# melspectrum007/audio-visual-speech-enhancement

Measured on AMD Instinct MI355X. Metric: clips/sec (STFT+CNN forward) on 200-ms@16kHz segments, 1/2/4/8 MI355X, higher is better.
Workload: dtype fp32_split

## Files before the change

audio-visual-speech-enhancement_amd/csrc/avse_common.h:

```cpp
#pragma once
#include <hip/hip_runtime.h>
#include <stdint.h>
#include <string>

#include "layer_geom.h"
#include "options.h"

typedef __bf16 bf16_t;
typedef __bf16 bf16x8 __attribute__((ext_vector_type(8)));
typedef _Float16 f16x8 __attribute__((ext_vector_type(8)));
typedef _Float16 f16x4 __attribute__((ext_vector_type(4)));
typedef float f32x4 __attribute__((ext_vector_type(4)));
typedef int i32x4 __attribute__((ext_vector_type(4)));

struct avse_ctx;

namespace avse {

void set_error(const std::string& msg);

int ctx_device_index(const struct ::avse_ctx* c);

int ensure_lds_attr(const void* fn, int bytes);

// ... 166 lines not shown
    const float* sh4;
    int nt4, kpad4;
    int pt4, pl4, rows4, pitch4;
    int dy4, dx4, nx4;
    const bf16_t* w5;
    const float* sc5;
    const float* sh5;
    int nt5[4], kpad5[4];
    int dy5[4], dx5[4], nx5[4];
    long long woff5[4];
    int pt5, pl5, rows5, pitch5;
    const float* w6;
    float b6;
    unsigned* range_flag;
    unsigned range_bit;
};
bool dec_tail_supported(const DecTailArgs& a);
bool dec_tail_s16_supported(const DecTailArgs& a);
int launch_dec_tail_s16(const DecTailArgs& a, hipStream_t s);

struct AudEncArgs {
    const float* mel;
    bf16_t* out;
    long long out_clip_stride;
    int N;
    const bf16_t* w1;
    const bf16_t* w2;
    const bf16_t* w3;
    const bf16_t* w4;
    const bf16_t* w5;
// ... 23 lines not shown
    const bf16_t* w;
    int M, N, kpad;
    const float* scale;
    const float* shift;
    int act;
    bf16_t* out;
    long long ldo;
    int out_off;
    int ksplit;
    float* partial;
    int* counters;
    int split;
    int slabs_per_split;
    unsigned* range_flag;
    unsigned range_bit;
};
int gemm_ksplit(int M, int N, int kpad, int cap);
int gemm_s16_ksplit(int N, int kpad, int* slabs_per_split);
size_t gemm_ws_bytes(int M, int N, int kpad, int cap);
int launch_gemm(const GemmArgs& g, int mode, hipStream_t s);
int launch_aud_enc(const AudEncArgs& a, hipStream_t s);
int launch_dec_tail(const DecTailArgs& a, hipStream_t s);

enum HaloOut { OUT_BF16 = 0, OUT_S16 = 1, OUT_F32 = 2 };

struct HaloArgs {
    int variant;
    const void* in;
    const float* video;
    const float* vmean;
// ... 48 lines not shown
```

audio-visual-speech-enhancement_amd/csrc/capi.hip:

```cpp
#include <algorithm>
#include <atomic>
#include <cmath>
#include <cstdio>
#include <cstdlib>
#include <cstring>
#include <mutex>
#include <set>
#include <string>
#include <utility>
#include <vector>

#include "../../include/avse.h"
#include "avse_common.h"
#include "netplan.h"
#include "spec_tables.h"
#include "weight_pack.h"

namespace avse {
static thread_local std::string g_err;
void set_error(const std::string& msg) { g_err = msg; }

int ensure_lds_attr(const void* fn, int bytes) {
    static std::mutex mu;
    static std::set<std::pair<const void*, int>> done;
// ... 104 lines not shown
    {"no_audenc", "AVSE_NO_AUDENC", &Options::no_audenc},
    {"no_dechead", "AVSE_NO_DECHEAD", &Options::no_dechead},
    {"no_dectail", "AVSE_NO_DECTAIL", &Options::no_dectail},
    {"unfused_tail", "AVSE_UNFUSED_TAIL", &Options::unfused_tail},
    {"no_halo", "AVSE_NO_HALO", &Options::no_halo},
    {"mfma32", "AVSE_MFMA32", &Options::mfma32},
    {"serial", "AVSE_SERIAL", &Options::serial},
    {"graph", "AVSE_GRAPH", &Options::graph},
    {"gemm_ksplit_cap", "AVSE_GEMM_KSPLIT", &Options::gemm_ksplit_cap},
    {"dense_istft", "AVSE_DENSE_ISTFT", &Options::dense_istft},
    {"no_act_scale", "AVSE_NO_ACT_SCALE", &Options::no_act_scale},
    {"no_win", "AVSE_NO_WIN", &Options::no_win},
    {"no_v1p", "AVSE_NO_V1P", &Options::no_v1p},
    {"no_a1valu", "AVSE_NO_A1VALU", &Options::no_a1valu},
    {"no_planar", "AVSE_NO_PLANAR", &Options::no_planar},
    {"side_prio", "AVSE_SIDE_PRIO", &Options::side_prio},
};

struct avse_weights {
    int dtype = 0;
    int device = 0;
    uint64_t serial = 0;
    NetPlan plan = kPlan25;
    GpuLayer layers[kNumLayers - 1];
    float* d6_w = nullptr;
    float d6_bias = 0.f;
    mutable std::atomic<void*> vzero_emb{nullptr};
    mutable std::mutex vzero_mu;
    mutable unsigned vzero_range = 0;
    int act_exp[kNumLayers] = {};
// ... 340 lines not shown
const char* avse_last_error(void) { return g_err.c_str(); }

int avse_ctx_create(int device, avse_ctx** out) {
    if (!out) return fail(AVSE_ERR_INVALID, "out is NULL");
    int n = 0;
    AVSE_HIP_CHECK(hipGetDeviceCount(&n));
    if (device < 0 || device >= n) return fail(AVSE_ERR_INVALID, "bad device index");
    AVSE_HIP_CHECK(hipSetDevice(device));
    avse_ctx* c = new avse_ctx();
    c->device = device;
    for (const OptionName& o : kOptionNames) {
        const char* e = std::getenv(o.env);
        if (e && *e) c->opt.*(o.field) = std::atoi(e);
    }
    if (hipMalloc((void**)&c->mse_partial, sizeof(float) * 256) != hipSuccess ||
        hipMalloc((void**)&c->gemm_counters, sizeof(int) * 8192) != hipSuccess ||
        hipMemset(c->gemm_counters, 0, sizeof(int) * 8192) != hipSuccess ||
        hipMalloc((void**)&c->range, sizeof(unsigned) * 4) != hipSuccess ||
        hipMemset(c->range, 0, sizeof(unsigned) * 4) != hipSuccess ||
        hipHostMalloc((void**)&c->range_host, sizeof(unsigned) * 4, hipHostMallocDefault) != hipSuccess) {
        (void)hipFree(c->mse_partial);
        (void)hipFree(c->gemm_counters);
        (void)hipFree(c->range);
        delete c;
        return fail(AVSE_ERR_OOM, "hipMalloc failed (ctx)");
    }
    *out = c;
    return 0;
}

void avse_ctx_destroy(avse_ctx* c) {
    if (!c) return;
// ... 335 lines not shown
        if (split) {
            g.split = 1;
            if (mode == 1) {
                g.ksplit = choose_ksplit(g.M, g.N, g.kpad, dt);
                g.slabs_per_split = g.ksplit > 1 ? kFp32Block : 0;
            } else {
                g.ksplit = gemm_s16_ksplit(g.N, g.kpad, &g.slabs_per_split);
            }
            g.range_flag = rflag;
            g.range_bit = 1u << li;
        } else {
            g.ksplit = gemm_ksplit(g.M, g.N, g.kpad, opt.gemm_ksplit_cap);
        }
        g.partial = reinterpret_cast<float*>(c->arena + part_off);
        g.counters = c->gemm_counters;
        return launch_gemm(g, mode, s);
    };
    auto ksplit = [&](ConvArgs& a, size_t partial_off) {
        if (a.nphase != 1) return;
        const int64_t M = (int64_t)a.N * a.Hq * a.Wq;
        a.ksplit = choose_ksplit(M, a.Co, a.ph[0].kpad, dt, a.ph[0].ntaps == 1, &a.ksplit_slabs);
        a.partial = reinterpret_cast<float*>(c->arena + partial_off);
    };
    auto L = [&](int i) -> const GpuLayer& { return W->layers[i]; };
    int stage = 0;
    auto mark = [&]() -> int {
        if (ev) AVSE_HIP_CHECK(hipEventRecord(ev[stage], s));
        ++stage;
        return 0;
    };
// ... 141 lines not shown
                             : conv_args(G, buf(a_in[i]), in_cs, buf(B_CAT), CAT, G.def.cout, 0, N);
        const int dti = pairs(a, i > 0, true, i);
        if ((rc = conv(a, dti, G, sa)) || (rc = mark())) return rc;
    }
    if (concurrent) AVSE_HIP_CHECK(hipEventRecord(c->join, sa));
    if (video) {
        if ((rc = video_encoder(video, vdt, vmean, vstd, N, off, buf(B_CAT)))) return rc;
    } else {
        const size_t es = dt == AVSE_BF16 ? 2 : 4;
        if ((rc = launch_broadcast_row(W->vzero_emb.load(std::memory_order_acquire), (char*)buf(B_CAT) + AEMB * es, N, 2048 * es, CAT * es, s))) return rc;
        if (split && W->vzero_range && rflag && (rc = launch_flag_or(rflag, W->vzero_range, s))) return rc;
        for (int k = 0; k < 6; ++k)
            if ((rc = mark())) return rc;
    }
    if (concurrent) AVSE_HIP_CHECK(hipStreamWaitEvent(s, c->join, 0));
    if (use_gemm) {
        if ((rc = gemm(L(11), buf(B_CAT), CAT, buf(B_E1), EMB, 0, 0, N, off[B_COUNT], 11)) || (rc = mark())) return rc;
        if ((rc = gemm(L(12), buf(B_E1), EMB, buf(B_E2), EMB, 0, 0, N, off[B_COUNT], 12)) || (rc = mark())) return rc;
        if ((rc = gemm(L(13), buf(B_E2), EMB, buf(B_E3), AEMB, 0, 0, N, off[B_COUNT], 13)) || (rc = mark())) return rc;
    } else {
        ConvArgs a = conv_args(L(11), buf(B_CAT), CAT, buf(B_E1), EMB, EMB, 0, N);
        ksplit(a, off[B_COUNT]);
        int dti = pairs(a, true, true, 11);
        if ((rc = launch_conv(a, split ? dti : cdt, s)) || (rc = mark())) return rc;
        a = conv_args(L(12), buf(B_E1), EMB, buf(B_E2), EMB, EMB, 0, N);
        ksplit(a, off[B_COUNT]);
        dti = pairs(a, true, true, 12);
        if ((rc = launch_conv(a, split ? dti : cdt, s)) || (rc = mark())) return rc;
        a = conv_args(L(13), buf(B_E2), EMB, buf(B_E3), AEMB, AEMB, 0, N);
        ksplit(a, off[B_COUNT]);
        dti = pairs(a, true, true, 13);
        if ((rc = launch_conv(a, split ? dti : cdt, s)) || (rc = mark())) return rc;
    }
    const int d_in[6] = {B_E3, B_D1, B_D2, B_D3, B_D4, B_D5};
    for (int i = 0; i < 5; ++i) {
        const GpuLayer& G = L(14 + i);
        const long long in_cs = (long long)G.def.hin * G.def.win * G.def.cin;
        if (i == 0 && dt == AVSE_BF16) {
            auto taps_ok = [&](const GpuLayer& D, int np, int nt, bool wide) {
                if (D.nphase != np || D.def.cin != 128 || D.def.cout != 128) return false;
                for (int p = 0; p < np; ++p) {
                    if (D.ph[p].ntaps != nt || D.ph[p].kpad != nt * 128 || D.ph[p].w_off != (long long)p * 128 * nt * 128) return false;
                    for (int t = 0; t < nt; ++t) {
                        const int2 d = D.htaps[D.ph[p].tap_off + t];
                        const int dy = wide ? (p >> 1) - (t >> 1) : 0, dx = wide ? (p & 1) - (t & 1) : -t;
                        if (d.x != dy || d.y != dx) return false;
                    }
// ... 10 lines not shown
            ha.out = reinterpret_cast<bf16_t*>(buf(B_D3));
            ha.out_clip_stride = 40 * 10 * 128;
            ha.N = (int)N;
            ha.w1 = (const bf16_t*)L(14).w; ha.w2 = (const bf16_t*)L(15).w; ha.w3 = (const bf16_t*)L(16).w;
            for (int k = 0; k < 3; ++k) { ha.sc[k] = L(14 + k).scale; ha.sh[k] = L(14 + k).shift; }
            if (shapes && !opt.no_dechead && dec_head_supported(ha)) {
                if ((rc = launch_dec_head(ha, s)) || (rc = mark()) || (rc = mark()) || (rc = mark())) return rc;
                i = 2;
                continue;
            }
        }
        if (i == 3 && split && !opt.unfused_tail && !opt.no_dectail) {
            DecTailArgs da = dec_tail_args(L(17), L(18), W, buf(d_in[3]), out, N);
            da.range_flag = rflag;
            da.range_bit = 1u << 17;
            if (dec_tail_s16_supported(da)) {
                if ((rc = launch_dec_tail_s16(da, s)) || (rc = mark()) || (rc = mark())) return rc;
                break;
            }
        }
        if (i == 3 && dt == AVSE_BF16 && !opt.unfused_tail && !opt.no_dectail) {
            const DecTailArgs da = dec_tail_args(L(17), L(18), W, buf(d_in[3]), out, N);
            if (dec_tail_supported(da)) {
                if ((rc = launch_dec_tail(da, s)) || (rc = mark()) || (rc = mark())) return rc;
                break;
            }
        }
        if (i == 4 && !opt.unfused_tail) {
            ConvArgs a = conv_args(G, buf(d_in[i]), in_cs, nullptr, (long long)G.ho * G.wo, 1, 0, N);
            a.fuse_w = W->d6_w;
// ... 247 lines not shown
```

audio-visual-speech-enhancement_amd/csrc/conv_dects.hip:

```cpp
#include <cstdlib>
#include <utility>

#include "avse_common.h"

namespace avse {
namespace {

#ifndef AVSE_DECTS_ABL
#define AVSE_DECTS_ABL 0
#endif
constexpr int DABL = AVSE_DECTS_ABL;
constexpr float LRELU = 0.3f;
constexpr int kOOB = 0x7fffff00;
constexpr int H = 40, W = 10;
constexpr int CI4 = 128, CO = 64;
constexpr int NW = 8, NT = 64 * NW;
constexpr int R4 = 21;
constexpr int F4 = 14, F5 = 13, SL = 7;
constexpr int P4 = 18, S4 = 96, ROWS4 = 26, WBUF = ROWS4 * P4 * S4;
constexpr int LROWS4 = 24, LCOLS4 = 14, NPC = 3;
constexpr int P5 = 18, S5 = 288, ROWS5 = 23, OIMG = ROWS5 * P5 * S5;
constexpr int REGION = ((OIMG > 2 * WBUF ? OIMG : 2 * WBUF) + 1023) / 1024 * 1024;
constexpr int BOFF = REGION;
constexpr int PAR = BOFF + 2 * 4 * 4096;
constexpr int PSC4 = PAR, PSH4 = PAR + 256, PSC5 = PAR + 512, PSH5 = PAR + 768, PW6 = PAR + 1024;
constexpr int XP = PAR + 1280;
constexpr int LDS_BYTES = XP + 4 * 16 * F5 * 4;
static_assert(LDS_BYTES <= 160 * 1024, "LDS");
static_assert(2 * SL == F4 && 16 * F4 >= R4 * W && 16 * F5 >= H / 2 * W && 16 * (F5 - 1) < H / 2 * W, "fragments");

constexpr int ph_ny(int p) { return 2 + (p >> 1); }
constexpr int ph_nx(int p) { return 2 + (p & 1); }
constexpr int ph_nt(int p) { return ph_ny(p) * ph_nx(p); }
constexpr int ph_woff(int p) { int s = 0; for (int q = 0; q < p; ++q) s += CO * ph_nt(q) * CO; return s; }
constexpr int ph_gstart(int p) { int s = 0; for (int q = 0; q < p; ++q) s += 4 * ph_nt(q); return s; }
constexpr int ph_of(int g) { int p = 0; while (p < 3 && g >= ph_gstart(p + 1)) ++p; return p; }
static_assert(ph_gstart(4) % 4 == 0 && (4 * ph_nt(0)) % 4 == 0, "every phase is whole ring groups");

__device__ __forceinline__ __amdgpu_buffer_rsrc_t make_rsrc(const void* base, long long bytes) {
    const int nrec = bytes > kOOB ? kOOB : (bytes < 0 ? 0 : (int)bytes);
    return __builtin_amdgcn_make_buffer_rsrc(const_cast<void*>(base), (short)0, nrec, 0x00020000);
}
__device__ __forceinline__ int wsw(int row) { return 2 * ((row >> 2) & 1); }
__device__ __forceinline__ i32x4 lds16(const char* base, int off) { return *reinterpret_cast<const i32x4*>(base + off); }
typedef int i32x2 __attribute__((ext_vector_type(2)));
__device__ __forceinline__ float bn_lrelu(float acc, float sc, float sh) {
    const float v = fmaf(acc, sc, sh);
    return fmaxf(v, LRELU * v);
}
__device__ __forceinline__ void lds_barrier_raw() {
    asm volatile("s_waitcnt lgkmcnt(0)" ::: "memory");
    asm volatile("s_barrier" ::: "memory");
}
__device__ __forceinline__ void lds_barrier() { lds_barrier_raw(); }
__device__ __forceinline__ void loop_barrier() {
    if constexpr (!(DABL & 4)) lds_barrier_raw();
}
template <int... I, typename F>
__device__ __forceinline__ void unroll(std::integer_sequence<int, I...>, F&& f) {
    (f(std::integral_constant<int, I>{}), ...);
}

__global__ __launch_bounds__(NT, 1) void k_dec_tail_s16(DecTailArgs a) {
    extern __shared__ __attribute__((aligned(1024))) char lds[];

    const int tid = threadIdx.x, lane = tid & 63;
    const int w = __builtin_amdgcn_readfirstlane(tid >> 6);
    const int r16 = lane & 15, kg = lane >> 4;
    const int clip = blockIdx.x >> 1, half = blockIdx.x & 1;
    const int cb = w & 3, fr0 = SL * (w >> 2);
    const bool s6 = w < 4;

    const int brow = tid >> 3, kq = (tid >> 1) & 3, kh = tid & 1;
    const int bst = BOFF + brow * 64 + ((kq ^ wsw(brow)) << 4) + kh * 8;
    const int brd = 16 * cb + r16;
    const int bfh = BOFF + brd * 64 + (((kg & 1) ^ wsw(brd)) << 4);
    const int bfl = BOFF + brd * 64 + (((2 + (kg & 1)) ^ wsw(brd)) << 4);
    auto st8 = [&](int addr, i32x2 v) { *reinterpret_cast<i32x2*>(lds + addr) = v; };
    auto read_w = [&](int off, i32x4 (&f)[2]) {
        f[0] = lds16(lds, bfh + off);
        f[1] = lds16(lds, bfl + off);
    };

    f32x4 acc[SL], part[SL];
    auto zero_all = [&]() {
#pragma unroll
        for (int i = 0; i < SL; ++i) acc[i] = part[i] = (f32x4){0.f, 0.f, 0.f, 0.f};
    };
    auto flush = [&]() {
#pragma unroll
        for (int i = 0; i < SL; ++i) {
            acc[i] += part[i];
            part[i] = (f32x4){0.f, 0.f, 0.f, 0.f};
        }
    };
    auto mfma_all = [&](const i32x4 (&fa)[SL], const i32x4 (&fw)[2], bool slot6) {
        if constexpr (DABL & 1) {
#pragma unroll
            for (int i = 0; i < SL; ++i) asm volatile("" ::"v"(fa[i]));
            asm volatile("" ::"v"(fw[0]), "v"(fw[1]));
            return;
        }
#pragma unroll
        for (int i = 0; i < SL; ++i) {
            if (i == SL - 1 && !slot6) continue;
            part[i] = __builtin_amdgcn_mfma_f32_16x16x32_f16(__builtin_bit_cast(f16x8, fw[0]), __builtin_bit_cast(f16x8, fa[i]),
                                                             part[i], 0, 0, 0);
            part[i] = __builtin_amdgcn_mfma_f32_16x16x32_f16(__builtin_bit_cast(f16x8, fw[1]), __builtin_bit_cast(f16x8, fa[i]),
                                                             part[i], 0, 0, 0);
        }
    };
// ... 22 lines not shown
            pok[k] = p < LROWS4 * LCOLS4;
            const bool in = pok[k] && iy >= 0 && iy < H && ix >= 0 && ix < W;
            psrc[k] = in ? ((iy * W + ix) * CI4 * 2 + sg * 8) * 2 : kOOB;
            pdst[k] = (wr * P4 + wc) * S4 + sg * 16;
        }
        const __amdgpu_buffer_rsrc_t rsW = make_rsrc(a.w4, (long long)CO * 16 * CI4 * 4);
        const int vbl = brow * (16 * CI4 * 4) + kq * 16 + kh * 8;
        auto bpiece = [&](auto tt, int csoff) {
            constexpr int t = decltype(tt)::value;
            return __builtin_amdgcn_raw_buffer_load_b64(rsW, vbl + t * 512, csoff, 0);
        };
        int vb[SL];
#pragma unroll
        for (int i = 0; i < SL; ++i) {
            const int q = 16 * (fr0 + i) + r16, r = q / W, x = q - r * W;
            vb[i] = (r * P4 + x) * S4 + kg * 16;
        }
        {
            i32x4 pc[NPC];
#pragma unroll
            for (int k = 0; k < NPC; ++k) pc[k] = __builtin_amdgcn_raw_buffer_load_b128(rsIn, psrc[k], 0, 0);
#pragma unroll
            for (int k = 0; k < NPC; ++k)
                if (pok[k]) *reinterpret_cast<i32x4*>(lds + pdst[k]) = pc[k];
        }
        i32x2 pb[4];
        {
            i32x2 w0[4];
            unroll(std::make_integer_sequence<int, 4>{}, [&](auto tt) {
                constexpr int t = decltype(tt)::value;
                w0[t] = bpiece(tt, 0);
                pb[t] = bpiece(std::integral_constant<int, t + 4>{}, 0);
            });
#pragma unroll
            for (int t = 0; t < 4; ++t) st8(bst + t * 4096, w0[t]);
        }
        zero_all();
        lds_barrier();

        i32x4 fa[2][SL], fw[2][2];
        constexpr int PST = 12;
        i32x4 pr[NPC];
        int wb = 0;
        auto read_a = [&](auto tt, i32x4 (&f)[SL]) {
            constexpr int t = decltype(tt)::value % 16;
            constexpr int imm = ((3 - t / 4) * P4 + (3 - t % 4)) * S4;
#pragma unroll
            for (int i = 0; i < SL; ++i) f[i] = lds16(lds + imm + wb, vb[i]);
        };
        read_a(std::integral_constant<int, 0>{}, fa[0]);
        read_w(0, fw[0]);
        for (int c = 0; c < 8; ++c) {
            const int nb = (c & 1) ? 0 : WBUF;
            const int cs = c * 64, cn = (c + 1) * 64;
            unroll(std::make_integer_sequence<int, 16>{}, [&](auto tt) {
                constexpr int t = decltype(tt)::value;
                __builtin_amdgcn_sched_barrier(0);
                st8(bst + (((t / 4) + 1) & 1) * 16384 + (t % 4) * 4096, pb[t & 3]);
                if constexpr (t + 8 < 16) pb[t & 3] = bpiece(std::integral_constant<int, t + 8>{}, cs);
                else pb[t & 3] = bpiece(std::integral_constant<int, t + 8 - 16>{}, cn);
                if constexpr (t < NPC) pr[t] = __builtin_amdgcn_raw_buffer_load_b128(rsIn, psrc[t], cn, 0);
                if constexpr (t >= PST && t - PST < NPC) {
                    if (pok[t - PST] && c < 7) *reinterpret_cast<i32x4*>(lds + nb + pdst[t - PST]) = pr[t - PST];
                }
                if constexpr (t % 4 == 3) loop_barrier();
                if constexpr (t == 15) wb = nb;
                if constexpr (DABL & 2) {
                } else if constexpr (t < 15) {
                    read_a(std::integral_constant<int, t + 1>{}, fa[(t + 1) & 1]);
                } else if (c < 7) {
// ... 3 lines not shown
                __builtin_amdgcn_sched_barrier(0);
                mfma_all(fa[t & 1], fw[t & 1], true);
                if constexpr (t % 8 == 7) flush();
            });
        }
        lds_barrier();

        {
            const int zrow = half ? 21 : 0;
            for (int u = tid; u < (12 + 2 * 22) * 16; u += NT) {
                const int px = u >> 4, pc = u & 15;
                const int i = px < 12 ? zrow : (px - 12) >> 1, xi = px < 12 ? px : ((px - 12) & 1) * 11;
                *reinterpret_cast<i32x4*>(lds + (i * P5 + xi) * S5 + pc * 16) = (i32x4){0, 0, 0, 0};
            }
        }
        const f32x4 sc = par4(PSC4), sh = par4(PSH4);
#pragma unroll
        for (int i = 0; i < SL; ++i) {
            const int q = 16 * (fr0 + i) + r16;
            if (q >= R4 * W) continue;
            const int r = q / W, x = q - r * W;
            const int px = ((r + 1 - half) * P5 + x + 1) * S5 + cb * 64 + 8 * kg;
            f16x4 hv, lv;
#pragma unroll
            for (int e = 0; e < 4; ++e) {
                const float y = bn_lrelu(acc[i][e], sc[e], sh[e]);
                range_bad |= pair_out_of_range(y);
                hv[e] = (_Float16)y;
                lv[e] = (_Float16)(y - (float)hv[e]);
            }
            *reinterpret_cast<f16x4*>(lds + px) = hv;
            *reinterpret_cast<f16x4*>(lds + px + 32) = lv;
        }
        lds_barrier();
    }
    range_report(a.range_flag, a.range_bit, range_bad);

    float* const outc = a.out + (long long)clip * (4 * H * W);
    const __amdgpu_buffer_rsrc_t rsW5 = make_rsrc(a.w5, (long long)ph_woff(4) * 4);
    int vrow5[3];
    vrow5[0] = brow * (4 * CO * 4) + kq * 16 + kh * 8;
    vrow5[1] = brow * (6 * CO * 4) + kq * 16 + kh * 8;
    vrow5[2] = brow * (9 * CO * 4) + kq * 16 + kh * 8;
    auto bpiece5 = [&](auto gg) {
        constexpr int g = decltype(gg)::value < ph_gstart(4) ? decltype(gg)::value : ph_gstart(3);
        constexpr int p = ph_of(g), sl = g - ph_gstart(p);
        constexpr int kk = p == 0 ? 0 : p == 3 ? 2 : 1;
        return __builtin_amdgcn_raw_buffer_load_b64(rsW5, vrow5[kk], ph_woff(p) * 4 + sl * 64, 0);
    };
    int vb5[SL];
#pragma unroll
    for (int i = 0; i < SL; ++i) {
        const int q = 16 * (fr0 + i) + r16, yl = q / W, x = q - yl * W;
        vb5[i] = (yl * P5 + x) * S5 + kg * 16;
    }
    auto read_a5 = [&](auto gg, i32x4 (&f)[SL]) {
        constexpr int g = decltype(gg)::value;
        constexpr int p = ph_of(g), sl = g - ph_gstart(p), tap = sl / 4, c = sl % 4;
        constexpr int dy = (p >> 1) - tap / ph_nx(p), dx = (p & 1) - tap % ph_nx(p);
        constexpr int imm = ((dy + 1) * P5 + (dx + 1)) * S5 + c * 64;
#pragma unroll
        for (int i = 0; i < SL - 1; ++i) f[i] = lds16(lds + imm, vb5[i]);
        if (s6) f[SL - 1] = lds16(lds + imm, vb5[SL - 1]);
    };
    float* const xp = reinterpret_cast<float*>(lds + XP);
    auto epilogue5 = [&](auto pp) {
        constexpr int p = decltype(pp)::value, py = p >> 1, px = p & 1;
        flush();
        const f32x4 sc = par4(PSC5), sh = par4(PSH5), w6 = par4(PW6);
#pragma unroll
        for (int i = 0; i < SL; ++i) {
            if (i == SL - 1 && !s6) continue;
            float d = 0.f;
#pragma unroll
            for (int e = 0; e < 4; ++e) d = fmaf(bn_lrelu(acc[i][e], sc[e], sh[e]), w6[e], d);
            d += __shfl_xor(d, 16);
            d += __shfl_xor(d, 32);
            const int q = 16 * (fr0 + i) + r16;
            if (kg == 0 && q < H / 2 * W) xp[cb * (16 * F5) + q] = d;
// ... 8 lines not shown
    };

    i32x2 pb[4];
    {
        i32x2 w0[4];
        unroll(std::make_integer_sequence<int, 4>{}, [&](auto tt) {
            constexpr int t = decltype(tt)::value;
            w0[t] = bpiece5(tt);
            pb[t] = bpiece5(std::integral_constant<int, t + 4>{});
        });
#pragma unroll
        for (int t = 0; t < 4; ++t) st8(bst + t * 4096, w0[t]);
    }
    zero_all();
    lds_barrier();
    i32x4 fa[2][SL], fw[2][2];
    read_a5(std::integral_constant<int, 0>{}, fa[0]);
    read_w(0, fw[0]);
    unroll(std::make_integer_sequence<int, ph_gstart(4)>{}, [&](auto gg) {
        constexpr int g = decltype(gg)::value, p = ph_of(g);
        constexpr bool last = g + 1 == ph_gstart(p + 1);
        __builtin_amdgcn_sched_barrier(0);
        st8(bst + (((g / 4) + 1) & 1) * 16384 + (g % 4) * 4096, pb[g & 3]);
        pb[g & 3] = bpiece5(std::integral_constant<int, g + 8>{});
        if constexpr (g % 4 == 3) loop_barrier();
        if constexpr (!last && !(DABL & 2)) {
            read_a5(std::integral_constant<int, g + 1>{}, fa[(g + 1) & 1]);
            read_w((((g + 1) / 4) & 1) * 16384 + ((g + 1) % 4) * 4096, fw[(g + 1) & 1]);
        }
        __builtin_amdgcn_sched_barrier(0);
        mfma_all(fa[g & 1], fw[g & 1], s6);
        if constexpr (!last && (g - ph_gstart(p)) % 8 == 7) flush();
        if constexpr (last) {
            epilogue5(std::integral_constant<int, p>{});
// ... 6 lines not shown
}

}

bool dec_tail_s16_supported(const DecTailArgs& a) {
    if (a.N <= 0 || a.nt4 != 16 || a.kpad4 != 16 * CI4 || a.dy4 != 1 || a.dx4 != 1 || a.nx4 != 4) return false;
    if (a.pt4 != 2 || a.pl4 != 2 || a.pt5 != 1 || a.pl5 != 1) return false;
    for (int p = 0; p < 4; ++p)
        if (a.nt5[p] != ph_nt(p) || a.kpad5[p] != ph_nt(p) * CO || a.dy5[p] != (p >> 1) || a.dx5[p] != (p & 1) ||
            a.nx5[p] != ph_nx(p) || a.woff5[p] != ph_woff(p))
            return false;
    return true;
}

int launch_dec_tail_s16(const DecTailArgs& a, hipStream_t s) {
    if (int rc = ensure_lds_attr((const void*)k_dec_tail_s16, LDS_BYTES)) return rc;
    hipLaunchKernelGGL(k_dec_tail_s16, dim3(2 * a.N), dim3(NT), LDS_BYTES, s, a);
    AVSE_HIP_CHECK(hipGetLastError());
    return 0;
}

}
```

audio-visual-speech-enhancement_amd/csrc/gemm.hip:

```cpp
#include <algorithm>
#include <cstdlib>

#include "avse_common.h"

namespace avse {
namespace {

constexpr float LRELU = 0.3f;
constexpr int kOOB = 0x7fffff00;
constexpr int NT = 512;
constexpr int SLAB = 16384;
constexpr int GRP = 4 * SLAB;
constexpr int LDS_BYTES = 2 * GRP;

__device__ __forceinline__ __amdgpu_buffer_rsrc_t make_rsrc(const void* base, long long bytes) {
    const int nrec = bytes > kOOB ? kOOB : (bytes < 0 ? 0 : (int)bytes);
    return __builtin_amdgcn_make_buffer_rsrc(const_cast<void*>(base), (short)0, nrec, 0x00020000);
}
__device__ __forceinline__ int wsw(int row) { return 2 * ((row >> 2) & 1); }
__device__ __forceinline__ i32x4 lds16(const char* p) { return *reinterpret_cast<const i32x4*>(p); }

template <int MODE, int ABL = 0, bool S16 = false>
__global__ __launch_bounds__(NT, 1) void k_gemm(GemmArgs g) {
    extern __shared__ __attribute__((aligned(1024))) char lds[];
    __shared__ int last_flag;
    const int tid = threadIdx.x, lane = tid & 63;
    const int w = __builtin_amdgcn_readfirstlane(tid >> 6);
    const int r16 = lane & 15, kg = lane >> 4;
    const int wm = w >> 2, wn = w & 3;
    const int m0 = blockIdx.x * 128, n0 = blockIdx.y * 128, z = blockIdx.z;
    constexpr int KB = S16 ? 4 : 2;
    const int nslab_all = g.kpad * KB / 64;
    const int sps = S16 && g.slabs_per_split > 0 ? g.slabs_per_split : (nslab_all + g.ksplit - 1) / g.ksplit;
    const int s_begin = z * sps, nsl = min(nslab_all, s_begin + sps) - s_begin;

    const int lrow = tid >> 2, part = tid & 3;
    const int ldst = lrow * 64 + ((part ^ wsw(lrow)) << 4);
// ... 24 lines not shown
            va = __builtin_amdgcn_raw_buffer_load_b128(rsA, pad ? kOOB : avoff, sa * 64, 0);
        } else {
            const int tap = sa / CPT, c = sa % CPT, dy = tap / 3 - 1, dx = tap - 3 * (tap / 3) - 1;
            const bool ok = (unsigned)(py + dy) < 4u && (unsigned)(px + dx) < 4u && avoff != kOOB && !pad;
            va = __builtin_amdgcn_raw_buffer_load_b128(rsA, ok ? avoff + (dy * 4 + dx) * PIXB : kOOB, c * 64, 0);
        }
    };
    auto store = [&](int s, const i32x4& va, const i32x4& vw) {
        char* const d = lds + ((s >> 2) & 1) * GRP + (s & 3) * SLAB + ldst;
        *reinterpret_cast<i32x4*>(d) = va;
        *reinterpret_cast<i32x4*>(d + 8192) = vw;
    };
    const int afr = (64 * wm + r16) * 64 + ((kg ^ wsw(r16)) << 4);
    const int bfr = 8192 + (32 * wn + r16) * 64 + (((S16 ? kg & 1 : kg) ^ wsw(r16)) << 4);
    const int bfl = 8192 + (32 * wn + r16) * 64 + (((2 + (kg & 1)) ^ wsw(r16)) << 4);
    i32x4 fa[2][4], fb[2][2], fl[2][2];
    auto read = [&](int s, int buf) {
        const char* const b = lds + ((s >> 2) & 1) * GRP + (s & 3) * SLAB;
#pragma unroll
        for (int i = 0; i < 4; ++i) fa[buf][i] = lds16(b + afr + 1024 * i);
#pragma unroll
        for (int j = 0; j < 2; ++j) fb[buf][j] = lds16(b + bfr + 1024 * j);
        if constexpr (S16) {
#pragma unroll
            for (int j = 0; j < 2; ++j) fl[buf][j] = lds16(b + bfl + 1024 * j);
        }
    };
    f32x4 acc[4][2], blk[4][2];
#pragma unroll
    for (int i = 0; i < 4; ++i) acc[i][0] = acc[i][1] = blk[i][0] = blk[i][1] = (f32x4){0.f, 0.f, 0.f, 0.f};
    float esc[2], esh[2];
// ... 3 lines not shown
        esc[j] = n < g.N ? g.scale[n] : 0.f;
        esh[j] = n < g.N ? g.shift[n] : 0.f;
    }

    i32x4 ra[4], rw[4];
    {
        i32x4 a0[4], w0[4];
#pragma unroll
        for (int s = 0; s < 4; ++s) load(s, a0[s], w0[s]);
#pragma unroll
        for (int s = 0; s < 4; ++s) load(s + 4, ra[s], rw[s]);
#pragma unroll
        for (int s = 0; s < 4; ++s) store(s, a0[s], w0[s]);
    }
    __syncthreads();
    read(0, 0);
    if constexpr (S16) {
        const int npad8 = (nsl + kFp32Block - 1) & ~(kFp32Block - 1);
        for (int s0 = 0; s0 < npad8; s0 += kFp32Block) {
#pragma unroll
            for (int q = 0; q < kFp32Block; ++q) {
                const int s = s0 + q;
                __builtin_amdgcn_sched_barrier(0);
                store(s + 4, ra[q & 3], rw[q & 3]);
                load(s + 8, ra[q & 3], rw[q & 3]);
                if ((q & 3) == 3) __syncthreads();
                read(s + 1, (q + 1) & 1);
                __builtin_amdgcn_sched_barrier(0);
                if constexpr ((ABL & 4) != 0) {
#pragma unroll
                    for (int i = 0; i < 4; ++i)
                        blk[i][0][0] += __builtin_bit_cast(float, fa[q & 1][i][0] ^ fb[q & 1][i & 1][1] ^ fl[q & 1][i & 1][2]);
// ... 130 lines not shown

int gemm_s16_ksplit(int N, int kpad, int* slabs_per_split) {
    const int nblocks = (kpad / 16 + kFp32Block - 1) / kFp32Block, tiles_n = (N + 127) / 128;
    int ks = std::max(1, std::min(nblocks, 256 / (4 * tiles_n)));
    const int G = (nblocks + ks - 1) / ks;
    ks = (nblocks + G - 1) / G;
    if (slabs_per_split) *slabs_per_split = G * kFp32Block;
    return ks;
}

int launch_gemm(const GemmArgs& g, int mode, hipStream_t s) {
    const bool s16 = g.split != 0;
#ifndef AVSE_GEMM_ABL
#define AVSE_GEMM_ABL 0
#endif
    const void* kf = mode == 0 ? (s16 ? (const void*)k_gemm<0, AVSE_GEMM_ABL, true> : (const void*)k_gemm<0>)
                               : (s16 ? (const void*)k_gemm<1, AVSE_GEMM_ABL, true> : (const void*)k_gemm<1>);
    if (int rc = ensure_lds_attr(kf, LDS_BYTES)) return rc;
    const int kq = s16 ? 16 : 32;
    const int nslab = g.kpad / kq;
    const bool s16_bad = s16 && (g.N % 16 || (g.ksplit > 1 && (g.slabs_per_split <= 0 || g.slabs_per_split % kFp32Block ||
                                                               (nslab + g.slabs_per_split - 1) / g.slabs_per_split != g.ksplit)));
    if (g.kpad % kq || g.M <= 0 || g.N <= 0 || g.ksplit < 1 || (g.ksplit > 1 && (!g.partial || !g.counters)) ||
        (mode == 1 && (g.M % 16 || g.kpad != 9 * 512)) || s16_bad) {
        set_error("gemm: bad arguments");
        return 3;
    }
    const dim3 grid((g.M + 127) / 128, (g.N + 127) / 128, g.ksplit);
    hipLaunchKernelGGL(reinterpret_cast<void (*)(GemmArgs)>(const_cast<void*>(kf)), grid, dim3(NT), LDS_BYTES, s, g);
    AVSE_HIP_CHECK(hipGetLastError());
    return 0;
}

}
```

audio-visual-speech-enhancement_amd/csrc/layer_geom.h:

```cpp
#pragma once
#include <utility>
#include <vector>

#include "netplan.h"

namespace avse {

constexpr int MAX_TAPS = 25;
constexpr int MAX_PHASES = 4;

struct ConvPhase {
    int py, px;
    int ntaps;
    int kpad;
    long long w_off;
    int tap_off;
};

struct Tap {
    int dy, dx;
};

inline long long kidx(const LayerDef& L, int ky, int kx, int ci, int co) {
    if (L.kind == DENSE) return (long long)ci * L.cout + co;
// ... 137 lines not shown
inline std::vector<int> gather_map(const LayerDef& L, const PhaseSet& g) {
    std::vector<int> m((size_t)g.w_elems, -1);
    for (int p = 0; p < g.nphase; ++p)
        for (int n = 0; n < g.rows; ++n) {
            int* row = m.data() + (size_t)g.ph[p].w_off + (size_t)n * g.ph[p].kpad;
            for (size_t j = 0; j < g.kyx[p].size(); ++j) {
                const int ky = g.kyx[p][j].first, kx = g.kyx[p][j].second;
                const long long k0 = g.dgrad ? kidx(L, ky, kx, n, 0) : kidx(L, ky, kx, 0, n);
                const long long dk = (g.dgrad ? kidx(L, ky, kx, n, 1) : kidx(L, ky, kx, 1, n)) - k0;
                for (int c = 0; c < g.red; ++c) row[j * g.cp + c] = (int)(k0 + c * dk);
            }
        }
    return m;
}

}
```

audio-visual-speech-enhancement_amd/csrc/options.h:

```cpp
#pragma once

namespace avse {

struct Options {
    int no_gemm = 0;
    int no_audenc = 0;
    int no_dechead = 0;
    int no_dectail = 0;
    int unfused_tail = 0;
    int no_halo = 0;
    int mfma32 = 0;
    int serial = 0;
    int graph = 0;
    int gemm_ksplit_cap = 0;
    int dense_istft = 0;
    int no_act_scale = 0;
    int no_win = 0;
    int no_v1p = 0;
    int no_a1valu = 0;
    int no_planar = 0;
    int side_prio = 0;
};

enum HaloVariant { HALO_NONE = -1, HALO_V1 = 0, HALO_K5 = 1, HALO_K3_16 = 2, HALO_K3_8 = 3, HALO_V1P = 4 };

}
```

Before: 82730.

## Fuse split-fp16 hi/lo operand pairs to cut MFMA products in s16 GEMM and decoder tail

For the split-fp16 (s16) path, hi and lo halves of the activations and weights now sit in paired slab layouts, so the GEMM issues three products (hi*hi, lo*hi, hi*lo) and the decoder tail issues the lo-activation product fused with the hi pair, replacing the old four-product schedule. Both kernels are templated on the new mode, which is on by default, with an env option to fall back to four products. Fewer MFMAs per k-slab cut matrix-core work on the fp32-emulation path. Dropping the lo*lo term may cost some accuracy. A counters-capacity check lets oversized GEMMs fall back to the conv path, and the dense-layer dispatch is folded into a loop.

```diff
diff --git a/audio-visual-speech-enhancement_amd/csrc/avse_common.h b/audio-visual-speech-enhancement_amd/csrc/avse_common.h
--- a/audio-visual-speech-enhancement_amd/csrc/avse_common.h
+++ b/audio-visual-speech-enhancement_amd/csrc/avse_common.h
@@ -204,6 +204,7 @@
     float b6;
     unsigned* range_flag;
     unsigned range_bit;
+    int four_products;
 };
 bool dec_tail_supported(const DecTailArgs& a);
 bool dec_tail_s16_supported(const DecTailArgs& a);
@@ -257,6 +258,8 @@
     int slabs_per_split;
     unsigned* range_flag;
     unsigned range_bit;
+    int counters_cap;
+    int four_products;
 };
 int gemm_ksplit(int M, int N, int kpad, int cap);
 int gemm_s16_ksplit(int N, int kpad, int* slabs_per_split);
diff --git a/audio-visual-speech-enhancement_amd/csrc/capi.hip b/audio-visual-speech-enhancement_amd/csrc/capi.hip
--- a/audio-visual-speech-enhancement_amd/csrc/capi.hip
+++ b/audio-visual-speech-enhancement_amd/csrc/capi.hip
@@ -142,6 +142,7 @@
     {"no_v1p", "AVSE_NO_V1P", &Options::no_v1p},
     {"no_a1valu", "AVSE_NO_A1VALU", &Options::no_a1valu},
     {"no_planar", "AVSE_NO_PLANAR", &Options::no_planar},
+    {"four_products", "AVSE_FOUR_PRODUCTS", &Options::four_products},
     {"side_prio", "AVSE_SIDE_PRIO", &Options::side_prio},
 };
 
@@ -512,8 +513,8 @@
         if (e && *e) c->opt.*(o.field) = std::atoi(e);
     }
     if (hipMalloc((void**)&c->mse_partial, sizeof(float) * 256) != hipSuccess ||
-        hipMalloc((void**)&c->gemm_counters, sizeof(int) * 8192) != hipSuccess ||
-        hipMemset(c->gemm_counters, 0, sizeof(int) * 8192) != hipSuccess ||
+        hipMalloc((void**)&c->gemm_counters, sizeof(int) * kGemmCounters) != hipSuccess ||
+        hipMemset(c->gemm_counters, 0, sizeof(int) * kGemmCounters) != hipSuccess ||
         hipMalloc((void**)&c->range, sizeof(unsigned) * 4) != hipSuccess ||
         hipMemset(c->range, 0, sizeof(unsigned) * 4) != hipSuccess ||
         hipHostMalloc((void**)&c->range_host, sizeof(unsigned) * 4, hipHostMallocDefault) != hipSuccess) {
@@ -879,6 +880,8 @@
         }
         g.partial = reinterpret_cast<float*>(c->arena + part_off);
         g.counters = c->gemm_counters;
+        g.counters_cap = kGemmCounters;
+        g.four_products = opt.four_products;
         return launch_gemm(g, mode, s);
     };
     auto ksplit = [&](ConvArgs& a, size_t partial_off) {
@@ -1050,23 +1053,17 @@
             if ((rc = mark())) return rc;
     }
     if (concurrent) AVSE_HIP_CHECK(hipStreamWaitEvent(s, c->join, 0));
-    if (use_gemm) {
-        if ((rc = gemm(L(11), buf(B_CAT), CAT, buf(B_E1), EMB, 0, 0, N, off[B_COUNT], 11)) || (rc = mark())) return rc;
-        if ((rc = gemm(L(12), buf(B_E1), EMB, buf(B_E2), EMB, 0, 0, N, off[B_COUNT], 12)) || (rc = mark())) return rc;
-        if ((rc = gemm(L(13), buf(B_E2), EMB, buf(B_E3), AEMB, 0, 0, N, off[B_COUNT], 13)) || (rc = mark())) return rc;
-    } else {
-        ConvArgs a = conv_args(L(11), buf(B_CAT), CAT, buf(B_E1), EMB, EMB, 0, N);
-        ksplit(a, off[B_COUNT]);
-        int dti = pairs(a, true, true, 11);
-        if ((rc = launch_conv(a, split ? dti : cdt, s)) || (rc = mark())) return rc;
-        a = conv_args(L(12), buf(B_E1), EMB, buf(B_E2), EMB, EMB, 0, N);
-        ksplit(a, off[B_COUNT]);
-        dti = pairs(a, true, true, 12);
-        if ((rc = launch_conv(a, split ? dti : cdt, s)) || (rc = mark())) return rc;
-        a = conv_args(L(13), buf(B_E2), EMB, buf(B_E3), AEMB, AEMB, 0, N);
-        ksplit(a, off[B_COUNT]);
-        dti = pairs(a, true, true, 13);
-        if ((rc = launch_conv(a, split ? dti : cdt, s)) || (rc = mark())) return rc;
+    const struct { int li, in, out; long long lda, ldo; } dense[3] = {
+        {11, B_CAT, B_E1, CAT, EMB}, {12, B_E1, B_E2, EMB, EMB}, {13, B_E2, B_E3, EMB, AEMB}};
+    for (const auto& d : dense) {
+        rc = use_gemm ? gemm(L(d.li), buf(d.in), d.lda, buf(d.out), d.ldo, 0, 0, N, off[B_COUNT], d.li) : -1;
+        if (rc == -1) {
+            ConvArgs a = conv_args(L(d.li), buf(d.in), d.lda, buf(d.out), d.ldo, d.ldo, 0, N);
+            ksplit(a, off[B_COUNT]);
+            const int dti = pairs(a, true, true, d.li);
+            rc = launch_conv(a, split ? dti : cdt, s);
+        }
+        if (rc || (rc = mark())) return rc;
     }
     const int d_in[6] = {B_E3, B_D1, B_D2, B_D3, B_D4, B_D5};
     for (int i = 0; i < 5; ++i) {
@@ -1107,6 +1104,7 @@
             DecTailArgs da = dec_tail_args(L(17), L(18), W, buf(d_in[3]), out, N);
             da.range_flag = rflag;
             da.range_bit = 1u << 17;
+            da.four_products = opt.four_products;
             if (dec_tail_s16_supported(da)) {
                 if ((rc = launch_dec_tail_s16(da, s)) || (rc = mark()) || (rc = mark())) return rc;
                 break;
diff --git a/audio-visual-speech-enhancement_amd/csrc/conv_dects.hip b/audio-visual-speech-enhancement_amd/csrc/conv_dects.hip
--- a/audio-visual-speech-enhancement_amd/csrc/conv_dects.hip
+++ b/audio-visual-speech-enhancement_amd/csrc/conv_dects.hip
@@ -36,6 +36,7 @@
 constexpr int ph_gstart(int p) { int s = 0; for (int q = 0; q < p; ++q) s += 4 * ph_nt(q); return s; }
 constexpr int ph_of(int g) { int p = 0; while (p < 3 && g >= ph_gstart(p + 1)) ++p; return p; }
 static_assert(ph_gstart(4) % 4 == 0 && (4 * ph_nt(0)) % 4 == 0, "every phase is whole ring groups");
+static_assert(ph_gstart(1) % 2 == 0 && ph_gstart(2) % 2 == 0 && ph_gstart(3) % 2 == 0, "every phase is whole slab pairs");
 
 __device__ __forceinline__ __amdgpu_buffer_rsrc_t make_rsrc(const void* base, long long bytes) {
     const int nrec = bytes > kOOB ? kOOB : (bytes < 0 ? 0 : (int)bytes);
@@ -61,6 +62,7 @@
     (f(std::integral_constant<int, I>{}), ...);
 }
 
+template <bool PR>
 __global__ __launch_bounds__(NT, 1) void k_dec_tail_s16(DecTailArgs a) {
     extern __shared__ __attribute__((aligned(1024))) char lds[];
 
@@ -73,9 +75,9 @@
 
     const int brow = tid >> 3, kq = (tid >> 1) & 3, kh = tid & 1;
     const int bst = BOFF + brow * 64 + ((kq ^ wsw(brow)) << 4) + kh * 8;
-    const int brd = 16 * cb + r16;
-    const int bfh = BOFF + brd * 64 + (((kg & 1) ^ wsw(brd)) << 4);
-    const int bfl = BOFF + brd * 64 + (((2 + (kg & 1)) ^ wsw(brd)) << 4);
+    const int brd = 16 * cb + r16, bps = PR ? (kg >> 1) * 4096 : 0;
+    const int bfh = BOFF + bps + brd * 64 + (((kg & 1) ^ wsw(brd)) << 4);
+    const int bfl = BOFF + bps + brd * 64 + (((2 + (kg & 1)) ^ wsw(brd)) << 4);
     auto st8 = [&](int addr, i32x2 v) { *reinterpret_cast<i32x2*>(lds + addr) = v; };
     auto read_w = [&](int off, i32x4 (&f)[2]) {
         f[0] = lds16(lds, bfh + off);
@@ -95,6 +97,36 @@
         }
     };
     auto mfma_all = [&](const i32x4 (&fa)[SL], const i32x4 (&fw)[2], bool slot6) {
+        if constexpr (DABL & 1) {
+#pragma unroll
+            for (int i = 0; i < SL; ++i) asm volatile("" ::"v"(fa[i]));
+            asm volatile("" ::"v"(fw[0]), "v"(fw[1]));
+            return;
+        }
+#pragma unroll
+        for (int i = 0; i < SL; ++i) {
+            if (i == SL - 1 && !slot6) continue;
+            part[i] = __builtin_amdgcn_mfma_f32_16x16x32_f16(__builtin_bit_cast(f16x8, fw[0]), __builtin_bit_cast(f16x8, fa[i]),
+                                                             part[i], 0, 0, 0);
+            part[i] = __builtin_amdgcn_mfma_f32_16x16x32_f16(__builtin_bit_cast(f16x8, fw[1]), __builtin_bit_cast(f16x8, fa[i]),
+                                                             part[i], 0, 0, 0);
+        }
+    };
+
+    auto mfma_l = [&](const i32x4 (&fl)[SL], const i32x4 (&fw)[2], bool slot6) {
+        if constexpr (DABL & 1) {
+#pragma unroll
+            for (int i = 0; i < SL; ++i) asm volatile("" ::"v"(fl[i]));
+            return;
+        }
+#pragma unroll
+        for (int i = 0; i < SL; ++i) {
+            if (i == SL - 1 && !slot6) continue;
+            part[i] = __builtin_amdgcn_mfma_f32_16x16x32_f16(__builtin_bit_cast(f16x8, fw[0]), __builtin_bit_cast(f16x8, fl[i]),
+                                                             part[i], 0, 0, 0);
+        }
+    };
+    auto mfma_h = [&](const i32x4 (&fa)[SL], const i32x4 (&fw)[2], bool slot6) {
         if constexpr (DABL & 1) {
 #pragma unroll
             for (int i = 0; i < SL; ++i) asm volatile("" ::"v"(fa[i]));
@@ -147,7 +179,7 @@
 #pragma unroll
         for (int i = 0; i < SL; ++i) {
             const int q = 16 * (fr0 + i) + r16, r = q / W, x = q - r * W;
-            vb[i] = (r * P4 + x) * S4 + kg * 16;
+            vb[i] = (r * P4 + x) * S4 + (PR ? (kg & 1) * 16 - (kg >> 1) * S4 : kg * 16);
         }
         {
             i32x4 pc[NPC];
@@ -171,8 +203,8 @@
         zero_all();
         lds_barrier();
 
-        i32x4 fa[2][SL], fw[2][2];
-        constexpr int PST = 12;
+        i32x4 fa[2][SL], fl[SL], fw[2][2];
+        constexpr int PST = PR ? 4 : 12;
         i32x4 pr[NPC];
         int wb = 0;
         auto read_a = [&](auto tt, i32x4 (&f)[SL]) {
@@ -181,12 +213,56 @@
 #pragma unroll
             for (int i = 0; i < SL; ++i) f[i] = lds16(lds + imm + wb, vb[i]);
         };
+        auto read_ap = [&](auto tt, auto hl, i32x4 (&f)[SL]) {
+            constexpr int t = decltype(tt)::value % 16;
+            constexpr int imm = ((3 - t / 4) * P4 + (3 - t % 4)) * S4 + 32 * decltype(hl)::value;
+#pragma unroll
+            for (int i = 0; i < SL; ++i) f[i] = lds16(lds + imm + wb, vb[i]);
+        };
+        constexpr std::integral_constant<int, 0> kH{};
+        constexpr std::integral_constant<int, 1> kL{};
         read_a(std::integral_constant<int, 0>{}, fa[0]);
+        if constexpr (PR) read_ap(std::integral_constant<int, 0>{}, kL, fl);
         read_w(0, fw[0]);
         for (int c = 0; c < 8; ++c) {
             const int nb = (c & 1) ? 0 : WBUF;
             const int cs = c * 64, cn = (c + 1) * 64;
-            unroll(std::make_integer_sequence<int, 16>{}, [&](auto tt) {
+            if constexpr (PR) unroll(std::make_integer_sequence<int, 8>{}, [&](auto uu) {
+                constexpr int u = decltype(uu)::value, t = 2 * u;
+                __builtin_amdgcn_sched_barrier(0);
+                unroll(std::make_integer_sequence<int, 2>{}, [&](auto dd) {
+                    constexpr int tq = t + decltype(dd)::value;
+                    st8(bst + (((tq / 4) + 1) & 1) * 16384 + (tq % 4) * 4096, pb[tq & 3]);
+                    if constexpr (tq + 8 < 16) pb[tq & 3] = bpiece(std::integral_constant<int, tq + 8>{}, cs);
+                    else pb[tq & 3] = bpiece(std::integral_constant<int, tq + 8 - 16>{}, cn);
+                    if constexpr (tq < NPC) pr[tq] = __builtin_amdgcn_raw_buffer_load_b128(rsIn, psrc[tq], cn, 0);
+                    if constexpr (tq >= PST && tq - PST < NPC) {
+                        if (pok[tq - PST] && c < 7) *reinterpret_cast<i32x4*>(lds + nb + pdst[tq - PST]) = pr[tq - PST];
+                    }
+                });
+                if constexpr (t % 4 == 2) loop_barrier();
+                if constexpr (t == 14) wb = nb;
+                if constexpr (DABL & 2) {
+                } else if constexpr (t < 14) {
+                    read_ap(std::integral_constant<int, t + 2>{}, kH, fa[(u + 1) & 1]);
+                } else if (c < 7) {
+                    read_ap(std::integral_constant<int, 0>{}, kH, fa[0]);
+                }
+                if constexpr (!(DABL & 2)) read_w((((t + 2) / 4) & 1) * 16384 + ((t + 2) % 4) * 4096, fw[(u + 1) & 1]);
+                __builtin_amdgcn_sched_barrier(0);
+                mfma_l(fl, fw[u & 1], true);
+                __builtin_amdgcn_sched_barrier(0);
+                if constexpr (DABL & 2) {
+                } else if constexpr (t < 14) {
+                    read_ap(std::integral_constant<int, t + 2>{}, kL, fl);
+                } else if (c < 7) {
+                    read_ap(std::integral_constant<int, 0>{}, kL, fl);
+                }
+                __builtin_amdgcn_sched_barrier(0);
+                mfma_h(fa[u & 1], fw[u & 1], true);
+                if constexpr (t % 8 == 6) flush();
+            });
+            else unroll(std::make_integer_sequence<int, 16>{}, [&](auto tt) {
                 constexpr int t = decltype(tt)::value;
                 __builtin_amdgcn_sched_barrier(0);
                 st8(bst + (((t / 4) + 1) & 1) * 16384 + (t % 4) * 4096, pb[t & 3]);
@@ -220,13 +296,15 @@
                 *reinterpret_cast<i32x4*>(lds + (i * P5 + xi) * S5 + pc * 16) = (i32x4){0, 0, 0, 0};
             }
         }
+        int lane4 = lane;
+        asm volatile("" : "+v"(lane4));
         const f32x4 sc = par4(PSC4), sh = par4(PSH4);
 #pragma unroll
         for (int i = 0; i < SL; ++i) {
-            const int q = 16 * (fr0 + i) + r16;
+            const int q = 16 * (fr0 + i) + (lane4 & 15);
             if (q >= R4 * W) continue;
             const int r = q / W, x = q - r * W;
-            const int px = ((r + 1 - half) * P5 + x + 1) * S5 + cb * 64 + 8 * kg;
+            const int px = ((r + 1 - half) * P5 + x + 1) * S5 + cb * 64 + 8 * (lane4 >> 4);
             f16x4 hv, lv;
 #pragma unroll
             for (int e = 0; e < 4; ++e) {
@@ -244,10 +322,13 @@
 
     float* const outc = a.out + (long long)clip * (4 * H * W);
     const __amdgpu_buffer_rsrc_t rsW5 = make_rsrc(a.w5, (long long)ph_woff(4) * 4);
+    int tid5 = tid;
+    asm volatile("" : "+v"(tid5));
+    const int r16_5 = tid5 & 15, kg_5 = (tid5 >> 4) & 3, brow5 = tid5 >> 3, kq5 = (tid5 >> 1) & 3, kh5 = tid5 & 1;
     int vrow5[3];
-    vrow5[0] = brow * (4 * CO * 4) + kq * 16 + kh * 8;
-    vrow5[1] = brow * (6 * CO * 4) + kq * 16 + kh * 8;
-    vrow5[2] = brow * (9 * CO * 4) + kq * 16 + kh * 8;
+    vrow5[0] = brow5 * (4 * CO * 4) + kq5 * 16 + kh5 * 8;
+    vrow5[1] = brow5 * (6 * CO * 4) + kq5 * 16 + kh5 * 8;
+    vrow5[2] = brow5 * (9 * CO * 4) + kq5 * 16 + kh5 * 8;
     auto bpiece5 = [&](auto gg) {
         constexpr int g = decltype(gg)::value < ph_gstart(4) ? decltype(gg)::value : ph_gstart(3);
         constexpr int p = ph_of(g), sl = g - ph_gstart(p);
@@ -257,8 +338,8 @@
     int vb5[SL];
 #pragma unroll
     for (int i = 0; i < SL; ++i) {
-        const int q = 16 * (fr0 + i) + r16, yl = q / W, x = q - yl * W;
-        vb5[i] = (yl * P5 + x) * S5 + kg * 16;
+        const int q = 16 * (fr0 + i) + r16_5, yl = q / W, x = q - yl * W;
+        vb5[i] = (yl * P5 + x) * S5 + (PR ? (kg_5 & 1) * 16 + (kg_5 >> 1) * 64 : kg_5 * 16);
     }
     auto read_a5 = [&](auto gg, i32x4 (&f)[SL]) {
         constexpr int g = decltype(gg)::value;
@@ -269,6 +350,18 @@
         for (int i = 0; i < SL - 1; ++i) f[i] = lds16(lds + imm, vb5[i]);
         if (s6) f[SL - 1] = lds16(lds + imm, vb5[SL - 1]);
     };
+    auto read_a5p = [&](auto gg, auto hl, i32x4 (&f)[SL]) {
+        constexpr int g = decltype(gg)::value;
+        constexpr int p = ph_of(g), sl = g - ph_gstart(p), tap = sl / 4, c = sl % 4;
+        static_assert(c % 2 == 0, "a pair lies inside one tap");
+        constexpr int dy = (p >> 1) - tap / ph_nx(p), dx = (p & 1) - tap % ph_nx(p);
+        constexpr int imm = ((dy + 1) * P5 + (dx + 1)) * S5 + c * 64 + 32 * decltype(hl)::value;
+#pragma unroll
+        for (int i = 0; i < SL - 1; ++i) f[i] = lds16(lds + imm, vb5[i]);
+        if (s6) f[SL - 1] = lds16(lds + imm, vb5[SL - 1]);
+    };
+    constexpr std::integral_constant<int, 0> kH{};
+    constexpr std::integral_constant<int, 1> kL{};
     float* const xp = reinterpret_cast<float*>(lds + XP);
     auto epilogue5 = [&](auto pp) {
         constexpr int p = decltype(pp)::value, py = p >> 1, px = p & 1;
@@ -307,10 +400,41 @@
     }
     zero_all();
     lds_barrier();
-    i32x4 fa[2][SL], fw[2][2];
+    i32x4 fa[2][SL], fl[SL], fw[2][2];
     read_a5(std::integral_constant<int, 0>{}, fa[0]);
+    if constexpr (PR) read_a5p(std::integral_constant<int, 0>{}, kL, fl);
     read_w(0, fw[0]);
-    unroll(std::make_integer_sequence<int, ph_gstart(4)>{}, [&](auto gg) {
+    if constexpr (PR) unroll(std::make_integer_sequence<int, ph_gstart(4) / 2>{}, [&](auto uu) {
+        constexpr int u = decltype(uu)::value, g = 2 * u, p = ph_of(g);
+        constexpr bool last = g + 2 == ph_gstart(p + 1);
+        __builtin_amdgcn_sched_barrier(0);
+        unroll(std::make_integer_sequence<int, 2>{}, [&](auto dd) {
+            constexpr int gq = g + decltype(dd)::value;
+            st8(bst + (((gq / 4) + 1) & 1) * 16384 + (gq % 4) * 4096, pb[gq & 3]);
+            pb[gq & 3] = bpiece5(std::integral_constant<int, gq + 8>{});
+        });
+        if constexpr (g % 4 == 2) loop_barrier();
+        if constexpr (!last && !(DABL & 2)) {
+            read_a5p(std::integral_constant<int, g + 2>{}, kH, fa[(u + 1) & 1]);
+            read_w((((g + 2) / 4) & 1) * 16384 + ((g + 2) % 4) * 4096, fw[(u + 1) & 1]);
+        }
+        __builtin_amdgcn_sched_barrier(0);
+        mfma_l(fl, fw[u & 1], s6);
+        __builtin_amdgcn_sched_barrier(0);
+        if constexpr (!last && !(DABL & 2)) read_a5p(std::integral_constant<int, g + 2>{}, kL, fl);
+        __builtin_amdgcn_sched_barrier(0);
+        mfma_h(fa[u & 1], fw[u & 1], s6);
+        if constexpr (!last && (g - ph_gstart(p)) % 8 == 6) flush();
+        if constexpr (last) {
+            epilogue5(std::integral_constant<int, p>{});
+            if constexpr (p < 3) {
+                read_a5p(std::integral_constant<int, g + 2>{}, kH, fa[(u + 1) & 1]);
+                read_a5p(std::integral_constant<int, g + 2>{}, kL, fl);
+                read_w((((g + 2) / 4) & 1) * 16384 + ((g + 2) % 4) * 4096, fw[(u + 1) & 1]);
+            }
+        }
+    });
+    else unroll(std::make_integer_sequence<int, ph_gstart(4)>{}, [&](auto gg) {
         constexpr int g = decltype(gg)::value, p = ph_of(g);
         constexpr bool last = g + 1 == ph_gstart(p + 1);
         __builtin_amdgcn_sched_barrier(0);
@@ -347,8 +471,9 @@
 }
 
 int launch_dec_tail_s16(const DecTailArgs& a, hipStream_t s) {
-    if (int rc = ensure_lds_attr((const void*)k_dec_tail_s16, LDS_BYTES)) return rc;
-    hipLaunchKernelGGL(k_dec_tail_s16, dim3(2 * a.N), dim3(NT), LDS_BYTES, s, a);
+    auto* const kf = a.four_products ? k_dec_tail_s16<false> : k_dec_tail_s16<true>;
+    if (int rc = ensure_lds_attr((const void*)kf, LDS_BYTES)) return rc;
+    hipLaunchKernelGGL(kf, dim3(2 * a.N), dim3(NT), LDS_BYTES, s, a);
     AVSE_HIP_CHECK(hipGetLastError());
     return 0;
 }
diff --git a/audio-visual-speech-enhancement_amd/csrc/gemm.hip b/audio-visual-speech-enhancement_amd/csrc/gemm.hip
--- a/audio-visual-speech-enhancement_amd/csrc/gemm.hip
+++ b/audio-visual-speech-enhancement_amd/csrc/gemm.hip
@@ -20,7 +20,7 @@
 __device__ __forceinline__ int wsw(int row) { return 2 * ((row >> 2) & 1); }
 __device__ __forceinline__ i32x4 lds16(const char* p) { return *reinterpret_cast<const i32x4*>(p); }
 
-template <int MODE, int ABL = 0, bool S16 = false>
+template <int MODE, int ABL = 0, bool S16 = false, bool PR = S16>
 __global__ __launch_bounds__(NT, 1) void k_gemm(GemmArgs g) {
     extern __shared__ __attribute__((aligned(1024))) char lds[];
     __shared__ int last_flag;
@@ -75,7 +75,21 @@
     const int afr = (64 * wm + r16) * 64 + ((kg ^ wsw(r16)) << 4);
     const int bfr = 8192 + (32 * wn + r16) * 64 + (((S16 ? kg & 1 : kg) ^ wsw(r16)) << 4);
     const int bfl = 8192 + (32 * wn + r16) * 64 + (((2 + (kg & 1)) ^ wsw(r16)) << 4);
-    i32x4 fa[2][4], fb[2][2], fl[2][2];
+    const int pso = (kg >> 1) * SLAB;
+    const int pah = pso + (64 * wm + r16) * 64 + (((kg & 1) ^ wsw(r16)) << 4);
+    const int pal = pso + (64 * wm + r16) * 64 + (((2 + (kg & 1)) ^ wsw(r16)) << 4);
+    i32x4 fa[2][4], fb[2][2], fl[2][2], fal[2][4];
+    auto read_pair = [&](int s, int buf) {
+        const char* const b = lds + ((s >> 2) & 1) * GRP + (s & 3) * SLAB;
+#pragma unroll
+        for (int i = 0; i < 4; ++i) fa[buf][i] = lds16(b + pah + 1024 * i);
+#pragma unroll
+        for (int i = 0; i < 4; ++i) fal[buf][i] = lds16(b + pal + 1024 * i);
+#pragma unroll
+        for (int j = 0; j < 2; ++j) fb[buf][j] = lds16(b + pso + bfr + 1024 * j);
+#pragma unroll
+        for (int j = 0; j < 2; ++j) fl[buf][j] = lds16(b + pso + bfl + 1024 * j);
+    };
     auto read = [&](int s, int buf) {
         const char* const b = lds + ((s >> 2) & 1) * GRP + (s & 3) * SLAB;
 #pragma unroll
@@ -109,8 +123,48 @@
         for (int s = 0; s < 4; ++s) store(s, a0[s], w0[s]);
     }
     __syncthreads();
-    read(0, 0);
-    if constexpr (S16) {
+    if constexpr (S16 && PR) read_pair(0, 0);
+    else read(0, 0);
+    if constexpr (S16 && PR) {
+        const int npad8 = (nsl + kFp32Block - 1) & ~(kFp32Block - 1);
+        for (int s0 = 0; s0 < npad8; s0 += kFp32Block) {
+#pragma unroll
+            for (int p = 0; p < kFp32Block / 2; ++p) {
+                const int s = s0 + 2 * p, q0 = (2 * p) & 3, q1 = (2 * p + 1) & 3;
+                __builtin_amdgcn_sched_barrier(0);
+                store(s + 4, ra[q0], rw[q0]);
+                load(s + 8, ra[q0], rw[q0]);
+                store(s + 5, ra[q1], rw[q1]);
+                load(s + 9, ra[q1], rw[q1]);
+                if (p & 1) __syncthreads();
+                read_pair(s + 2, (p + 1) & 1);
+                __builtin_amdgcn_sched_barrier(0);
+                if constexpr ((ABL & 4) != 0) {
+#pragma unroll
+                    for (int i = 0; i < 4; ++i)
+                        blk[i][0][0] += __builtin_bit_cast(float, fa[p & 1][i][0] ^ fal[p & 1][i][3] ^ fb[p & 1][i & 1][1] ^
+                                                                      fl[p & 1][i & 1][2]);
+                    continue;
+                }
+#pragma unroll
+                for (int h = 0; h < 3; ++h)
+#pragma unroll
+                    for (int i = 0; i < 4; ++i)
+#pragma unroll
+                        for (int j = 0; j < 2; ++j)
+                            blk[i][j] = __builtin_amdgcn_mfma_f32_16x16x32_f16(
+                                __builtin_bit_cast(f16x8, h == 1 ? fal[p & 1][i] : fa[p & 1][i]),
+                                __builtin_bit_cast(f16x8, h == 2 ? fl[p & 1][j] : fb[p & 1][j]), blk[i][j], 0, 0, 0);
+            }
+#pragma unroll
+            for (int i = 0; i < 4; ++i)
+#pragma unroll
+                for (int j = 0; j < 2; ++j) {
+                    acc[i][j] += blk[i][j];
+                    blk[i][j] = (f32x4){0.f, 0.f, 0.f, 0.f};
+                }
+        }
+    } else if constexpr (S16) {
         const int npad8 = (nsl + kFp32Block - 1) & ~(kFp32Block - 1);
         for (int s0 = 0; s0 < npad8; s0 += kFp32Block) {
 #pragma unroll
@@ -271,8 +325,13 @@
 #ifndef AVSE_GEMM_ABL
 #define AVSE_GEMM_ABL 0
 #endif
-    const void* kf = mode == 0 ? (s16 ? (const void*)k_gemm<0, AVSE_GEMM_ABL, true> : (const void*)k_gemm<0>)
-                               : (s16 ? (const void*)k_gemm<1, AVSE_GEMM_ABL, true> : (const void*)k_gemm<1>);
+    const bool pr = s16 && !g.four_products;
+    const void* kf = mode == 0 ? (pr    ? (const void*)k_gemm<0, AVSE_GEMM_ABL, true, true>
+                                  : s16 ? (const void*)k_gemm<0, AVSE_GEMM_ABL, true, false>
+                                        : (const void*)k_gemm<0>)
+                               : (pr    ? (const void*)k_gemm<1, AVSE_GEMM_ABL, true, true>
+                                  : s16 ? (const void*)k_gemm<1, AVSE_GEMM_ABL, true, false>
+                                        : (const void*)k_gemm<1>);
     if (int rc = ensure_lds_attr(kf, LDS_BYTES)) return rc;
     const int kq = s16 ? 16 : 32;
     const int nslab = g.kpad / kq;
@@ -283,6 +342,7 @@
         set_error("gemm: bad arguments");
         return 3;
     }
+    if (!gemm_tickets_fit(g.M, g.N, g.ksplit, g.counters_cap)) return -1;
     const dim3 grid((g.M + 127) / 128, (g.N + 127) / 128, g.ksplit);
     hipLaunchKernelGGL(reinterpret_cast<void (*)(GemmArgs)>(const_cast<void*>(kf)), grid, dim3(NT), LDS_BYTES, s, g);
     AVSE_HIP_CHECK(hipGetLastError());
diff --git a/audio-visual-speech-enhancement_amd/csrc/layer_geom.h b/audio-visual-speech-enhancement_amd/csrc/layer_geom.h
--- a/audio-visual-speech-enhancement_amd/csrc/layer_geom.h
+++ b/audio-visual-speech-enhancement_amd/csrc/layer_geom.h
@@ -175,4 +175,9 @@
     return m;
 }
 
+constexpr int kGemmCounters = 8192;
+inline bool gemm_tickets_fit(long long M, long long N, int ksplit, long long counters) {
+    return ksplit <= 1 || ((M + 127) / 128) * ((N + 127) / 128) <= counters;
 }
+
+}
diff --git a/audio-visual-speech-enhancement_amd/csrc/options.h b/audio-visual-speech-enhancement_amd/csrc/options.h
--- a/audio-visual-speech-enhancement_amd/csrc/options.h
+++ b/audio-visual-speech-enhancement_amd/csrc/options.h
@@ -19,6 +19,7 @@
     int no_v1p = 0;
     int no_a1valu = 0;
     int no_planar = 0;
+    int four_products = 0;
     int side_prio = 0;
 };
 
```

Result: faster. 85100 (median of 6 runs) (+2.9%).
